# Ezreal11/EaBNet

Hardware: AMD Instinct MI355X
Metric: enhanced frames/sec (16 kHz, 8-mic) at 1/2/4/8 MI355X; RTF per utterance (higher is better)
Workload: dtype f32; 1 GPU; BASELINE configs[1]/[2]: batch of 16 four-second 8-mic 16 kHz utterances per GPU, wave -> STFT+compress -> EaBNet.forward, inference, full hand-written HIP path; batch_per_gpu=16, global_batch=16, mics=8, frames_per_utt=401, freq_bins=161, parallelism=dp1 (independent shards, no collective), pipeline_depth=3

## Files before the change

eabnet_amd/_lib.py:

```python
from __future__ import annotations

import ctypes as C
import os
from typing import Optional

_HERE = os.path.dirname(os.path.abspath(__file__))
LIB_PATH = os.path.join(_HERE, "lib", "libeabnet_hip.so")
ABI_VERSION = 10
MAX_TAPS = 16
_fp = C.POINTER(C.c_float)


class TimeWindow(C.Structure):
    _fields_ = [("pos", C.c_void_p), ("count", C.c_int32), ("lens", C.c_void_p)]


class ConvDesc(C.Structure):
    _fields_ = [
        ("src0", C.c_void_p), ("src1", C.c_void_p), ("xf0", C.c_void_p), ("xf1", C.c_void_p),
        ("slope0", C.c_void_p), ("slope1", C.c_void_p),
        ("C0", C.c_int32), ("C1", C.c_int32), ("xf_mode", C.c_int32),
        ("w", C.c_void_p), ("bias", C.c_void_p),
        ("N", C.c_int32), ("Kpad", C.c_int32),
        ("B", C.c_int32), ("T", C.c_int32), ("Fin", C.c_int32), ("Fout", C.c_int32),
# ... 63 lines not shown
                            + [C.c_void_p] * 4),
    "eab_si_sdr_loss_bwd_f32": (C.c_int, [C.c_void_p, C.c_longlong, C.c_int] * 2 + [C.c_void_p, C.c_int, C.c_void_p, C.c_void_p,
                                          C.c_int, C.c_double, C.c_void_p, C.c_longlong, C.c_void_p]),
    "eab_mrstft_workspace_bytes": (C.c_longlong, [C.c_void_p] + [C.c_int] * 4),
    "eab_mrstft_loss_f32": (C.c_int, [C.c_void_p, C.c_longlong, C.c_int] * 2 + [C.c_void_p, C.c_int, C.c_void_p, C.c_int, C.c_void_p]
                            + [C.c_double] * 3 + [C.c_void_p, C.c_longlong] + [C.c_void_p] * 4),
    "eab_mrstft_loss_bwd_f32": (C.c_int, [C.c_void_p, C.c_longlong, C.c_int] * 2 + [C.c_void_p, C.c_int, C.c_void_p, C.c_int, C.c_void_p,
                                          C.c_double, C.c_void_p, C.c_void_p, C.c_int, C.c_double, C.c_void_p, C.c_longlong,
                                          C.c_void_p, C.c_longlong, C.c_void_p]),
    "eab_norm_act_win_f32": (C.c_int, [C.c_void_p] * 7 + [C.c_int] * 4 + [TimeWindow, C.c_void_p]),
    "eab_lstm64_stream_f32": (C.c_int, [C.c_void_p] * 3 + [C.c_float] + [C.c_void_p] * 4 + [C.c_int] * 4
                              + [TimeWindow, C.c_void_p]),
    "eab_bfw_filter_sum_win_f32": (C.c_int, [C.c_void_p] * 6 + [C.c_int] * 4 + [TimeWindow, C.c_void_p]),
    "eab_mlp_bfw_filter_sum_f32": (C.c_int, [C.c_void_p] * 8 + [C.c_int] * 4 + [TimeWindow, C.c_void_p]),
    "eab_zero_rows_f32": (C.c_int, [C.c_void_p] + [C.c_int] * 3 + [TimeWindow, C.c_void_p]),
    "eab_shift_rows_f32": (C.c_int, [C.c_void_p] + [C.c_int] * 5 + [C.c_void_p]),
    "eab_com_mag_mse_loss_f32": (C.c_int, [C.c_void_p] * 3 + [C.c_int] * 3 + [C.c_void_p, C.c_int, C.c_void_p, C.c_void_p,
                                            C.c_void_p]),
    "eab_energy_ratios_f32": (C.c_int, [C.c_void_p, C.c_longlong, C.c_int] * 3 + [C.c_void_p, C.c_int, C.c_void_p, C.c_int,
                                        C.c_void_p, C.c_void_p]),
    "eab_com_mag_mse_loss_lens_f32": (C.c_int, [C.c_void_p] * 3 + [C.c_int] * 4 + [C.c_void_p, C.c_int, C.c_void_p, C.c_void_p]),
    "eab_stoi_frame_capacity": (C.c_int, [C.c_int]),
    "eab_stoi_workspace_bytes": (C.c_longlong, [C.c_int, C.c_int]),
    "eab_stoi_f32": (C.c_int, [C.c_void_p, C.c_longlong, C.c_int] * 2 + [C.c_void_p, C.c_int, C.c_void_p, C.c_longlong]
                     + [C.c_void_p] * 5),
    "eab_stoi_bwd_workspace_bytes": (C.c_longlong, [C.c_int, C.c_int]),
    "eab_stoi_bwd_f32": (C.c_int, [C.c_void_p, C.c_longlong, C.c_int, C.c_int, C.c_void_p, C.c_int, C.c_void_p, C.c_longlong,
                                   C.c_double, C.c_double, C.c_void_p, C.c_int, C.c_double, C.c_void_p, C.c_longlong, C.c_void_p,
                                   C.c_longlong, C.c_void_p]),
    "eab_resample_bwd_f32": (C.c_int, [C.c_void_p, C.c_longlong, C.c_int, C.c_void_p, C.c_int, C.c_int, C.c_void_p, C.c_longlong,
                                       C.c_int, C.c_void_p, C.c_void_p, C.c_int, C.c_int, C.c_int, C.c_void_p]),
    "eab_resample_f32": (C.c_int, [C.c_void_p, C.c_longlong, C.c_int, C.c_void_p, C.c_void_p, C.c_int, C.c_int,
                                   C.c_void_p, C.c_longlong, C.c_int, C.c_void_p, C.c_void_p, C.c_int, C.c_int, C.c_int,
                                   C.c_longlong, C.c_longlong, C.c_longlong, C.c_void_p]),
    "eab_room_gains_f32": (C.c_int, [C.c_void_p] + [C.c_int] * 3 + [C.c_void_p] * 2 + [C.c_double, C.c_void_p, C.c_int, C.c_void_p,
                                                                                       C.c_void_p]),
    "eab_room_rirs_f32": (C.c_int, [C.c_void_p] + [C.c_int] * 4 + [C.c_double, C.c_void_p, C.c_void_p]),
    "eab_room_rirs_tail_f32": (C.c_int, [C.c_void_p] + [C.c_int] * 4 + [C.c_double, C.c_void_p, C.c_void_p]),
    "eab_room_workspace_bytes": (C.c_longlong, [C.c_int] * 5),
    "eab_room_convolve_f32": (C.c_int, [C.c_void_p] + [C.c_int] * 3 + [C.c_void_p] * 5 + [C.c_int] * 2 + [C.c_void_p] * 2
                              + [C.c_longlong] + [C.c_void_p] * 3),
    "eab_grad_sumsq_f64": (C.c_int, [C.POINTER(OptimSegment), C.c_int, C.c_void_p, C.c_longlong, C.c_void_p]),
    "eab_adam_clip_f32": (C.c_int, [C.POINTER(OptimSegment), C.c_int, C.c_void_p, C.c_longlong] + [C.c_double] * 7
                          + [C.c_void_p, C.c_void_p]),
    "eab_gag_pack_f32": (C.c_int, [C.c_void_p] * 4 + [C.c_int] * 4 + [TimeWindow, C.c_void_p]),
    "eab_gag_crm_f32": (C.c_int, [C.c_void_p] * 6 + [C.c_int] * 6 + [TimeWindow, C.c_void_p]),
    "eab_gag_crm_bwd_f32": (C.c_int, [C.c_void_p] * 9 + [C.c_int] * 6 + [C.c_void_p]),
    "eab_conv_tiles": (C.c_int, [C.c_int] * 3),
    "eab_conv_f32": (C.c_int, [C.POINTER(ConvDesc), C.c_void_p]),
    "eab_train_cln_bwd_f32": (C.c_int, [C.c_void_p] * 11 + [C.c_int] * 5 + [C.c_void_p]),
    "eab_conv_st_chain_plan": (C.c_int, [C.POINTER(ConvDesc), C.c_int, C.POINTER(C.c_int), C.POINTER(C.c_int), C.POINTER(C.c_int)]),
    "eab_conv_st_chain_run": (C.c_int, [C.c_void_p, C.c_void_p, C.c_int, C.c_int, C.c_int, C.c_int, C.c_void_p]),
    "eab_conv_bf16": (C.c_int, [C.POINTER(ConvDesc), C.c_void_p]),
    "eab_lstm64_bf16": (C.c_int, [C.c_void_p] * 3 + [C.c_float] + [C.c_void_p] * 3 + [C.c_int] * 3 + [C.c_void_p]),
    "eab_in_finalize_f32": (C.c_int, [C.c_void_p] + [C.c_int] * 5 + [C.c_float] + [C.c_void_p] * 6 + [C.c_void_p]),
    "eab_norm_act_f32": (C.c_int, [C.c_void_p] * 7 + [C.c_int] * 3 + [C.c_void_p]),
    "eab_lstm64_f32": (C.c_int, [C.c_void_p] * 3 + [C.c_float] + [C.c_void_p] * 3 + [C.c_int] * 3 + [C.c_void_p]),
    "eab_lstm64_prec_f32": (C.c_int, [C.c_void_p] * 3 + [C.c_float] + [C.c_void_p] * 3 + [C.c_int] * 4 + [C.c_void_p]),
    "eab_bfw_filter_sum_f32": (C.c_int, [C.c_void_p] * 6 + [C.c_int] * 4 + [C.c_void_p]),
    "eab_run_program": (C.c_int, [C.POINTER(Op), C.c_int, C.c_void_p]),
    "eab_sizeof_conv_desc": (C.c_int, []),
    "eab_sizeof_op": (C.c_int, []),
    "eab_sizeof_wgrad_desc": (C.c_int, []),
    "eab_gather_f32": (C.c_int, [C.c_void_p] * 4 + [C.c_longlong, C.c_void_p]),
    "eab_train_in_stats_f32": (C.c_int, [C.c_void_p] * 2 + [C.c_int] * 3 + [C.c_float] + [C.c_void_p] * 4 + [C.c_void_p]),
    "eab_train_in1d_f32": (C.c_int, [C.c_void_p] * 2 + [C.c_int] * 3 + [C.c_float] + [C.c_void_p] * 5 + [C.c_void_p]),
    "eab_train_in1d_multi_f32": (C.c_int, [C.c_void_p] * 2 + [C.c_int] * 4 + [C.c_float] + [C.c_void_p] * 5 + [C.c_void_p]),
    "eab_train_norm_bwd_multi_f32": (C.c_int, [C.c_void_p] * 12 + [C.c_int] * 3 + [C.c_void_p]),
    "eab_in_finalize_mr_f32": (C.c_int, [C.c_void_p] + [C.c_int] * 5 + [C.c_float] + [C.c_void_p] * 8 + [C.c_void_p]),
    "eab_train_norm_act_f32": (C.c_int, [C.c_void_p] * 5 + [C.c_int] * 4 + [C.c_void_p]),
    "eab_train_norm_bwd_f32": (C.c_int, [C.c_void_p] * 12 + [C.c_int] * 4 + [C.c_void_p]),
    "eab_glu_bwd_f32": (C.c_int, [C.c_void_p] * 3 + [C.c_longlong, C.c_int, C.c_void_p]),
    "eab_glu_bwd_ex_f32": (C.c_int, [C.c_void_p] * 3 + [C.c_longlong, C.c_int, C.c_int, C.c_void_p]),
    "eab_gate_fwd_f32": (C.c_int, [C.c_void_p] * 3 + [C.c_longlong, C.c_void_p]),
    "eab_gate_bwd_f32": (C.c_int, [C.c_void_p] * 5 + [C.c_longlong, C.c_void_p]),
    "eab_add_f32": (C.c_int, [C.c_void_p] * 3 + [C.c_longlong, C.c_void_p]),
    "eab_copy_f32": (C.c_int, [C.c_void_p] * 2 + [C.c_longlong, C.c_void_p]),
    "eab_relu_bwd_f32": (C.c_int, [C.c_void_p] * 3 + [C.c_longlong, C.c_void_p]),
    "eab_colsum_f32": (C.c_int, [C.c_void_p] * 2 + [C.c_longlong, C.c_int, C.c_void_p]),
    "eab_filter_sum_bwd_f32": (C.c_int, [C.c_void_p] * 3 + [C.c_int] * 5 + [C.c_void_p]),
    "eab_filter_sum_ld_f32": (C.c_int, [C.c_void_p] * 3 + [C.c_int] * 5 + [C.c_void_p]),
    "eab_layernorm64_fwd_f32": (C.c_int, [C.c_void_p] * 3 + [C.c_float] + [C.c_void_p] * 2 + [C.c_longlong, C.c_void_p]),
    "eab_layernorm64_bwd_f32": (C.c_int, [C.c_void_p] * 7 + [C.c_longlong, C.c_void_p]),
    "eab_lstm64_train_fwd_f32": (C.c_int, [C.c_void_p] * 5 + [C.c_int] * 3 + [C.c_void_p]),
    "eab_lstm64_bwd_f32": (C.c_int, [C.c_void_p] * 4 + [C.c_int] * 3 + [C.c_void_p]),
    "eab_lstm64_train_fwd_prec_f32": (C.c_int, [C.c_void_p] * 5 + [C.c_int] * 4 + [C.c_void_p]),
    "eab_lstm64_bwd_prec_f32": (C.c_int, [C.c_void_p] * 4 + [C.c_int] * 4 + [C.c_void_p]),
    "eab_wgrad_f32": (C.c_int, [C.POINTER(WgradDesc), C.c_void_p]),
    "eab_wgrad_batchable": (C.c_int, [C.c_void_p, C.c_int, C.c_int]),
    "eab_wgrad_batch_f32": (C.c_int, [C.c_void_p, C.c_int, C.c_int, C.c_void_p]),
    "eab_lstm64_bwd_form": (C.c_int, [C.c_int] * 4),
    "eab_train_in_stats_lens_f32": (C.c_int, [C.c_void_p] * 2 + [C.c_int] * 3 + [C.c_float] + [C.c_void_p] * 4
                                    + [C.c_void_p, C.c_int, C.c_void_p]),
    "eab_train_in1d_lens_f32": (C.c_int, [C.c_void_p] * 2 + [C.c_int] * 3 + [C.c_float] + [C.c_void_p] * 5
                                + [C.c_void_p, C.c_int, C.c_void_p]),
    "eab_train_in1d_multi_lens_f32": (C.c_int, [C.c_void_p] * 2 + [C.c_int] * 4 + [C.c_float] + [C.c_void_p] * 5
                                      + [C.c_void_p, C.c_int, C.c_void_p]),
    "eab_train_norm_bwd_lens_f32": (C.c_int, [C.c_void_p] * 12 + [C.c_int] * 4 + [C.c_void_p, C.c_int, C.c_void_p]),
    "eab_train_norm_bwd_multi_lens_f32": (C.c_int, [C.c_void_p] * 12 + [C.c_int] * 3 + [C.c_void_p, C.c_int, C.c_void_p]),
    "eab_layernorm64_bwd_lens_f32": (C.c_int, [C.c_void_p] * 7 + [C.c_longlong, C.c_void_p, C.c_int, C.c_int, C.c_void_p]),
    "eab_lstm64_bwd_lens_f32": (C.c_int, [C.c_void_p] * 5 + [C.c_int] * 4 + [C.c_void_p]),
    "eab_filter_sum_ld_lens_f32": (C.c_int, [C.c_void_p] * 3 + [C.c_int] * 5 + [C.c_void_p, C.c_void_p]),
    "eab_wgrad_batch_lens_f32": (C.c_int, [C.c_void_p, C.c_int, C.c_int, C.c_void_p, C.c_void_p]),
    "eab_cln_stats_f32": (C.c_int, [C.c_void_p] * 2 + [C.c_int] * 4 + [C.c_float] + [C.c_void_p] * 3 + [TimeWindow, C.c_void_p]),
    "eab_cln_apply_f32": (C.c_int, [C.c_void_p] * 7 + [C.c_int] * 5 + [TimeWindow, C.c_void_p]),
    "eab_cln_step_f32": (C.c_int, [C.c_void_p] * 10 + [C.c_int] * 5 + [C.c_float, TimeWindow, C.c_void_p]),
# ... 36 lines not shown
```

eabnet_amd/csrc/conv_gemm.hip:

```cpp
#include "device.h"
#include <type_traits>

#define CG_THREADS 256

#define CG_PLAIN 0
#define CG_GLU 1
#define CG_DUAL 2
#define CG_PH2 3
#define CG_XFC 128

#define CG_PMAX 352

template <int MI, int NI, int KU, int MODE, bool PATCH, bool XFT>
struct CgSmem {
    static constexpr int BM = 64 * MI, BN = 64 * NI, LDK = 16 * KU + 4;
    static constexpr int NA = MODE == CG_DUAL ? 2 : 1;
    static constexpr int ATILE = BM * LDK;
    float a[PATCH ? CG_PMAX * LDK : NA * 2 * ATILE];
    float b[2][BN * LDK];
    float xft[2][CG_XFC][2];
    float xsl[2][CG_XFC];
    int dt[EAB_MAX_TAPS];
    int ioff[EAB_MAX_TAPS];
    int last;
    static constexpr int RW = MODE == CG_PH2 ? 2 : 1;
    __attribute__((aligned(16))) unsigned rtab_own[XFT ? BM * RW : 4];
    static_assert(XFT || sizeof(float) * 2 * CG_XFC * 2 >= sizeof(unsigned) * BM * RW, "row table inside xft");
};

__device__ __forceinline__ void cg_merge(float& n, float& mean, float& m2, float nb, float meanb, float m2b) {
    const float nt = n + nb;
    if (nt > 0.0f) {
        const float delta = meanb - mean;
        const float fb = nb / nt;
        mean = fmaf(delta, fb, mean);
        m2 = m2 + m2b + delta * delta * n * fb;
    }
    n = nt;
}

template <int MI, int NI, int KU, int MODE, int XF, bool VEC, int PREC, bool PATCH, bool WIDE = false>
__global__ __launch_bounds__(CG_THREADS, (MI == 2 && NI == 2 && KU == 1 && MODE == CG_GLU) ? 3 : (MODE == CG_PH2 ? 2 : 1)) void conv_gemm_kernel(const eab_conv_desc d) {
    static_assert(MODE != CG_PH2 || (PATCH && NI == 2), "phase-pair form: patch pipeline, one column block per phase and wave");
    static_assert(!PATCH || (KU == 1 && MODE != CG_DUAL && VEC), "patch mode: one unit per stage, single transform");
    constexpr bool H3 = PREC == EAB_PREC_F16X3;
    constexpr bool BF = PREC == EAB_PREC_BF16;
    constexpr bool PH2 = MODE == CG_PH2;
    constexpr bool GLU = MODE != CG_PLAIN;
    constexpr bool DUAL = MODE == CG_DUAL;
    using Smem = CgSmem<MI, NI, KU, MODE, PATCH, XF != EAB_XF_NONE>;
    constexpr int BM = Smem::BM, BN = Smem::BN, LDK = Smem::LDK;
    __shared__ __attribute__((aligned(16))) Smem sm;

    const int tid = threadIdx.x;
    const int lane = tid & 63, wave = tid >> 6;
    const int wm = wave >> 1, wn = wave & 1;
    const int li = lane & 31, lh = lane >> 5;

    const int t_lo = d.win.pos ? *d.win.pos : 0;
    int t_hi = d.win.pos ? (t_lo + d.win.count < d.T ? t_lo + d.win.count : d.T) : d.T;
    const int tiles_per_b = ((d.win.pos ? d.win.count : d.T) * d.No + BM - 1) / BM;
    unsigned vblk = blockIdx.x;
    if (gridDim.x >= 64) {
        const unsigned G = gridDim.x, G8 = G >> 3, rem = G & 7, xcd = vblk & 7, idx = vblk >> 3;
        vblk = xcd * G8 + (xcd < rem ? xcd : rem) + idx;
    }
    const int b = (int)(vblk / (unsigned)tiles_per_b);
    const int tile = (int)vblk - b * tiles_per_b;
    int t_src = d.T;
    if (d.win.lens) {
        t_src = min(t_src, d.win.lens[b]);
        t_hi = min(t_hi, t_src);
    }
    const int Q = t_hi * d.No;
    const int q0 = t_lo * d.No + tile * BM;
    const int n_blk = blockIdx.y * BN;
    const float inv_no = 1.0f / (float)d.No;

#pragma unroll
    for (int j = 0; j < EAB_MAX_TAPS; ++j)
        if (tid == j) {
            sm.dt[j] = d.dt[j];
            sm.ioff[j] = d.ioff[j];
        }

    const int Cout = d.Cout;
    const unsigned row_bytes = (unsigned)(d.Fout * Cout) * 4u, step_bytes = (unsigned)(d.ostride * Cout) * 4u;
    const unsigned phase_bytes = (unsigned)(d.ophase * Cout) * 4u, chan_bytes = (unsigned)Cout * 4u;
    unsigned* const rtab = XF != EAB_XF_NONE ? sm.rtab_own : reinterpret_cast<unsigned*>(&sm.xft[0][0][0]);
    if (tid < BM) {
        const int q = q0 + tid;
        const bool ok = q < Q;
        const int t = eab_div(ok ? q : 0, d.No, inv_no), o = (ok ? q : 0) - t * d.No;
        const unsigned off = ok ? (unsigned)t * row_bytes + (unsigned)o * step_bytes + phase_bytes : EAB_OOB;
        if constexpr (PH2)
            *reinterpret_cast<uint2*>(&rtab[2 * tid]) = make_uint2(off, (ok && 2 * o + 1 < d.Fout) ? off + chan_bytes : EAB_OOB);
        else
            rtab[tid] = off;
    }

    if (XF != EAB_XF_NONE) {
        const int k = tid >> 7, c = tid & (CG_XFC - 1);
        const int Ck = (k == 0 || DUAL) ? d.C0 : d.C1;
        const float* xfk = k == 0 ? d.xf0 : d.xf1;
        const float* slk = k == 0 ? d.slope0 : d.slope1;
        float sc = 1.0f, sh = 0.0f, sl = 1.0f;
        if (c < Ck) {
            if (d.fin_stats && k < d.fin_nsets) {
                const float* gm = k == 0 ? d.fin_gamma0 : d.fin_gamma1;
                const float* bt = k == 0 ? d.fin_beta0 : d.fin_beta1;
                double sn = 0.0, sm = 0.0, sq = 0.0;
                for (int t = 0; t < d.fin_tiles; ++t) {
                    const f32x4 v = *reinterpret_cast<const f32x4*>(
                        &d.fin_stats[((((size_t)b * d.fin_tiles + t) * d.fin_nsets + k) * d.C0 + c) * 4]);
                    const double n = (double)v[0], mu = (double)v[1];
                    sn += n;
                    sm = fma(n, mu, sm);
                    sq += fma(n * mu, mu, (double)v[2]);
                }
                const double mean = sn > 0.0 ? sm / sn : 0.0;
                double var = sn > 0.0 ? sq / sn - mean * mean : 0.0;
                if (var < 0.0) var = 0.0;
                const double scale = (double)gm[c] / sqrt(var + (double)d.fin_eps);
                sc = (float)scale;
                sh = (float)((double)bt[c] - mean * scale);
                sl = slk[c];
            } else if (xfk) {
                const float2 v = *reinterpret_cast<const float2*>(&xfk[((size_t)b * Ck + c) * 2]);
                sc = v.x;
                sh = v.y;
                sl = slk[c];
            }
        }
        sm.xft[k][c][0] = sc;
        sm.xft[k][c][1] = sh;
        sm.xsl[k][c] = sl;
    }

    const int Ctot = d.C0 + d.C1;
    const int UPT = (Ctot + 15) >> 4;
    const int NU = d.ntaps * UPT;
    static_assert(!WIDE || (PREC == EAB_PREC_BF16 && KU == 1 && VEC && !PATCH && XF == EAB_XF_NONE && MODE != CG_DUAL), "WIDE: see above");
    constexpr bool w0 = WIDE, w1 = WIDE;
    const int NS = (w0 || w1) ? d.ntaps * ((w0 ? d.C0 >> 5 : (d.C0 + 15) >> 4) + (d.C1 > 0 ? (w1 ? d.C1 >> 5 : (d.C1 + 15) >> 4) : 0))
                              : (NU + KU - 1) / KU;

    constexpr unsigned esz0 = WIDE ? 2u : 4u, esz1 = WIDE ? 2u : 4u;
    const unsigned bytes0 = (unsigned)d.T * d.Fin * d.C0 * esz0;
    const unsigned bytes1 = (unsigned)d.T * d.Fin * d.C1 * esz1;
    const __amdgpu_buffer_rsrc_t rs0 = __builtin_amdgcn_make_buffer_rsrc(
        const_cast<char*>(reinterpret_cast<const char*>(d.src0)) + (size_t)b * bytes0, 0, bytes0, 0x00020000);
    const __amdgpu_buffer_rsrc_t rs1 = __builtin_amdgcn_make_buffer_rsrc(
        const_cast<char*>(reinterpret_cast<const char*>(d.src1 ? d.src1 : d.src0)) + (d.src1 ? (size_t)b * bytes1 : 0), 0,
        d.src1 ? bytes1 : 0u, 0x00020000);

    const int srow = tid >> 2;
    const int skq = tid & 3;
    const float* wrow[NI];
#pragma unroll
    for (int p = 0; p < NI; ++p) wrow[p] = d.w + (size_t)(n_blk + srow + 64 * p) * d.Kpad + skq * 4;

    f32x16 acc[MI][NI];
#pragma unroll
    for (int mi = 0; mi < MI; ++mi)
#pragma unroll
        for (int ni = 0; ni < NI; ++ni)
#pragma unroll
            for (int r = 0; r < 16; ++r) acc[mi][ni][r] = 0.0f;

    auto lds_barrier = [] { asm volatile("s_waitcnt lgkmcnt(0)\n\ts_barrier" ::: "memory"); };

    __syncthreads();

    if (q0 < Q) {
    if constexpr (PATCH) {
        constexpr int PP = (CG_PMAX + 63) / 64;
        int dt_min = 0, io_min = 0, io_max = 0;
#pragma unroll
        for (int j = 0; j < EAB_MAX_TAPS; ++j)
            if (j < d.ntaps) {
                dt_min = d.dt[j] < dt_min ? d.dt[j] : dt_min;
                io_min = d.ioff[j] < io_min ? d.ioff[j] : io_min;
                io_max = d.ioff[j] > io_max ? d.ioff[j] : io_max;
            }
        const int halo_lo = -io_min;
        const int hi_need = (d.No - 1) * d.istride + io_max - (d.Fin - 1);
        const int Fp = d.Fin + halo_lo + (hi_need > 0 ? hi_need : 0);
        const float inv_fp = 1.0f / (float)Fp;
        const int t_first = eab_div(q0, d.No, inv_no);
        const int t_last = eab_div((q0 + BM < Q ? q0 + BM : (Q > q0 ? Q : q0 + 1)) - 1, d.No, inv_no);
        const int P = (t_last - t_first + 1 - dt_min) * Fp;

        const int d64 = eab_div(64, Fp, inv_fp), m64 = 64 - d64 * Fp;
        int p_tf[PP];
        bool p_ok[PP], p_all[PP];
        {
            const int tr = eab_div(srow, Fp, inv_fp);
            int f = srow - tr * Fp, t_in = t_first + dt_min + tr;
            int tf = t_in * d.Fin + f - halo_lo;
#pragma unroll
            for (int pp = 0; pp < PP; ++pp) {
                p_ok[pp] = p_all[pp] = false;
                p_tf[pp] = 0;
                if (64 * pp < P) {
                    p_ok[pp] = srow + 64 * pp < P && (unsigned)t_in < (unsigned)t_src && (unsigned)(f - halo_lo) < (unsigned)d.Fin;
                    if (XF != EAB_XF_NONE) p_all[pp] = __builtin_amdgcn_ballot_w64(p_ok[pp]) == __builtin_amdgcn_ballot_w64(true);
                    p_tf[pp] = tf;
                    f += m64;
                    t_in += d64;
                    tf += d64 * d.Fin + m64;
                    if (f >= Fp) {
                        f -= Fp;
                        ++t_in;
                        tf += d.Fin - Fp;
                    }
                }
            }
        }
        int fa[MI];
#pragma unroll
        for (int mi = 0; mi < MI; ++mi) {
            int q = q0 + (wm * MI + mi) * 32 + li;
            q = q < Q ? q : (Q > q0 ? Q - 1 : q0);
            const int t = eab_div(q, d.No, inv_no), o = q - t * d.No;
            fa[mi] = ((t - t_first - dt_min) * Fp + o * d.istride + halo_lo) * LDK + 4 * lh;
        }
        const int b_base = (wn * NI * 32 + li) * LDK + 4 * lh;

        f32x4 rp[PP];
        f32x4 rbw0[NI], rbw1[NI];
        int p_tc = 0;
        auto patch_fetch = [&](int chunk) {
            const int c0 = chunk << 4;
            const bool second = (d.C1 > 0) && (c0 >= d.C0);
            const int Cs = second ? d.C1 : d.C0;
            const int c = (second ? c0 - d.C0 : c0) + skq * 4;
            const bool cok = c < Cs;
            p_tc = ((second ? 1 : 0) << 8) | (cok ? c : 0);
#pragma unroll
            for (int pp = 0; pp < PP; ++pp) {
                if (64 * pp >= P) continue;
                const unsigned off = (p_ok[pp] && cok) ? (unsigned)((p_tf[pp] * Cs + c) * 4) : EAB_OOB;
                const u32x4 v = second ? __builtin_amdgcn_raw_buffer_load_b128(rs1, off, 0, 0)
                                       : __builtin_amdgcn_raw_buffer_load_b128(rs0, off, 0, 0);
                rp[pp] = __builtin_bit_cast(f32x4, v);
            }
// ... 764 lines not shown
                    cg_merge(n, mu, q, red[i1], red[i1 + 1], red[i1 + 2]);
                    *reinterpret_cast<f32x4*>(&d.stats[((tbase + s) * Cout + ch[c]) * 4]) = f32x4{n, mu, q, 0.0f};
                }
            }
        }
        if (d.fz_counter) {
            __threadfence();
            __syncthreads();
            if (tid == 0) sm.last = atomicAdd(&d.fz_counter[b], 1) == d.stat_tiles - 1;
            __syncthreads();
            if (sm.last) {
                __threadfence();
                const int nch = d.nsets * Cout;
                const int NSL = CG_THREADS / nch;
                const int e = tid % nch, slice = tid / nch;
                const int s = e / Cout, c = e - s * Cout;
                double* dred = reinterpret_cast<double*>(&sm.a[0]);
                double sn = 0.0, sm_ = 0.0, sq = 0.0;
                if (slice < NSL) {
                    const float* p = d.stats + (((size_t)b * d.stat_tiles) * d.nsets + s) * Cout * 4 + (size_t)c * 4;
                    const size_t stride = (size_t)d.nsets * Cout * 4;
                    for (int t = slice; t < d.stat_tiles; t += NSL) {
                        const f32x4 v = *reinterpret_cast<const f32x4*>(p + (size_t)t * stride);
                        const double n = (double)v[0], mu = (double)v[1];
                        sn += n;
                        sm_ = fma(n, mu, sm_);
                        sq += fma(n * mu, mu, (double)v[2]);
                    }
                    dred[(0 * NSL + slice) * nch + e] = sn;
                    dred[(1 * NSL + slice) * nch + e] = sm_;
                    dred[(2 * NSL + slice) * nch + e] = sq;
                }
                __syncthreads();
                if (slice == 0) {
                    sn = sm_ = sq = 0.0;
                    for (int k = 0; k < NSL; ++k) {
                        sn += dred[(0 * NSL + k) * nch + e];
                        sm_ += dred[(1 * NSL + k) * nch + e];
                        sq += dred[(2 * NSL + k) * nch + e];
                    }
                    const double mean = sn > 0.0 ? sm_ / sn : 0.0;
                    double var = sn > 0.0 ? sq / sn - mean * mean : 0.0;
                    if (var < 0.0) var = 0.0;
                    const float* gm = s == 0 ? d.fz_gamma0 : d.fz_gamma1;
                    const float* bt = s == 0 ? d.fz_beta0 : d.fz_beta1;
                    float* xf = s == 0 ? d.fz_xf0 : d.fz_xf1;
                    const double scale = (double)gm[c] / sqrt(var + (double)d.fz_eps);
                    *reinterpret_cast<float2*>(&xf[((size_t)b * Cout + c) * 2]) = make_float2((float)scale, (float)((double)bt[c] - mean * scale));
                }
                if (tid == 0) d.fz_counter[b] = 0;
            }
        }
    }
}

extern "C" int eab_conv_tiles(int T, int No, int bm) {
    if (T <= 0 || No <= 0 || (bm != 16 && bm != 32 && bm != 64 && bm != 128)) return -1;
    long long q = (long long)T * No;
    return (int)((q + bm - 1) / bm);
}

int eab_conv_st(const eab_conv_desc* d, hipStream_t s);

template <int MI, int NI, int KU, int MODE, int XF, bool VEC>
static int cg_launch(const eab_conv_desc* d, hipStream_t s) {
    constexpr int BM = 64 * MI, BN = 64 * NI;
    const int tiles = eab_conv_tiles(d->win.pos ? d->win.count : d->T, d->No, BM);
    dim3 grid((unsigned)(d->B * tiles), (unsigned)(d->N / BN));
    constexpr bool can_patch = KU == 1 && MODE != CG_DUAL && VEC && XF != EAB_XF_PRELU_NORM;
    if (d->korder == EAB_KORDER_CHUNK) {
        if constexpr (can_patch) {
            if (d->precision == EAB_PREC_F16X3)
                hipLaunchKernelGGL((conv_gemm_kernel<MI, NI, 1, MODE, XF, true, EAB_PREC_F16X3, true>), grid,
                                   dim3(CG_THREADS), 0, s, *d);
            else if (d->precision == EAB_PREC_BF16)
                hipLaunchKernelGGL((conv_gemm_kernel<MI, NI, 1, MODE, XF, true, EAB_PREC_BF16, true>), grid,
                                   dim3(CG_THREADS), 0, s, *d);
            else
                hipLaunchKernelGGL((conv_gemm_kernel<MI, NI, 1, MODE, XF, true, EAB_PREC_F32, true>), grid,
                                   dim3(CG_THREADS), 0, s, *d);
            EAB_RETURN_LAUNCH_STATUS();
        } else {
            return EAB_EUNSUPPORTED;
        }
    }
    if constexpr (MODE == CG_PH2) {
        return EAB_EUNSUPPORTED;
    } else {
    if (d->precision == EAB_PREC_F16X3) {
        if constexpr (VEC)
            hipLaunchKernelGGL((conv_gemm_kernel<MI, NI, KU, MODE, XF, VEC, EAB_PREC_F16X3, false>), grid,
                               dim3(CG_THREADS), 0, s, *d);
        else
            return EAB_EUNSUPPORTED;
    } else if (d->precision == EAB_PREC_BF16) {
        if constexpr (VEC) {
            if (d->src_bf16) {
                if constexpr (KU == 1 && XF == EAB_XF_NONE && MODE != CG_DUAL)
                    hipLaunchKernelGGL((conv_gemm_kernel<MI, NI, KU, MODE, XF, VEC, EAB_PREC_BF16, false, true>), grid,
                                       dim3(CG_THREADS), 0, s, *d);
                else
                    return EAB_EUNSUPPORTED;
            } else {
                hipLaunchKernelGGL((conv_gemm_kernel<MI, NI, KU, MODE, XF, VEC, EAB_PREC_BF16, false>), grid,
                                   dim3(CG_THREADS), 0, s, *d);
            }
        } else {
            return EAB_EUNSUPPORTED;
        }
    } else {
        hipLaunchKernelGGL((conv_gemm_kernel<MI, NI, KU, MODE, XF, VEC, EAB_PREC_F32, false>), grid, dim3(CG_THREADS), 0,
                           s, *d);
    }
    EAB_RETURN_LAUNCH_STATUS();
    }
}

static long long cg_patch_positions(const eab_conv_desc* d) {
    int dt_min = 0, io_min = 0, io_max = 0;
    for (int j = 0; j < d->ntaps; ++j) {
        dt_min = d->dt[j] < dt_min ? d->dt[j] : dt_min;
        io_min = d->ioff[j] < io_min ? d->ioff[j] : io_min;
        io_max = d->ioff[j] > io_max ? d->ioff[j] : io_max;
    }
    const int hi_need = (d->No - 1) * d->istride + io_max - (d->Fin - 1);
    const long long Fp = d->Fin - io_min + (hi_need > 0 ? hi_need : 0);
    const long long rows = (d->bm - 1) / d->No + 2 - dt_min;
    return rows * Fp;
}

template <int MI, int NI, int MODE, int XF, bool VEC>
static int cg_pick_ku(const eab_conv_desc* d, hipStream_t s, int ku) {
    if (ku == 4) {
        if constexpr (MI == 1 && MODE != CG_GLU && VEC) return cg_launch<MI, NI, 4, MODE, XF, VEC>(d, s);
        return EAB_EUNSUPPORTED;
    }
    if (ku == 2) {
        if constexpr (VEC && MODE != CG_DUAL) return cg_launch<MI, NI, 2, MODE, XF, VEC>(d, s);
        return EAB_EUNSUPPORTED;
    }
    return cg_launch<MI, NI, 1, MODE, XF, VEC>(d, s);
}

extern "C" int eab_conv_f32(const eab_conv_desc* d, eab_stream_t stream) {
    EAB_CHECK_ARG(d && d->src0 && d->w && d->dst);
    EAB_CHECK_ARG(d->B > 0 && d->T > 0 && d->Fin > 0 && d->Fout > 0 && d->No > 0);
    EAB_CHECK_ARG(d->C0 > 0 && d->C1 >= 0 && (d->C1 == 0) == (d->src1 == nullptr));
    EAB_CHECK_ARG(d->C1 == 0 || (d->C0 % 16) == 0);
    EAB_CHECK_ARG(d->ntaps > 0 && d->ntaps <= EAB_MAX_TAPS);
    EAB_CHECK_ARG(d->ostride >= 1 && d->istride >= 1 && d->ophase >= 0 && d->ophase < d->ostride);
    EAB_CHECK_ARG((d->No - 1) * d->ostride + d->ophase < d->Fout);
    const int upt = (d->C0 + d->C1 + 15) / 16;
    EAB_CHECK_ARG(d->Kpad == d->ntaps * upt * 16);
    for (int j = 0; j < d->ntaps; ++j) {
        EAB_CHECK_ARG(d->dt[j] < (1 << 20) && d->dt[j] > -(1 << 20));
        EAB_CHECK_ARG(d->dt[j] <= 0 || d->korder != EAB_KORDER_CHUNK);
    }
    EAB_CHECK_ARG(d->epi >= EAB_EPI_LINEAR && d->epi <= EAB_EPI_PHASE2);
    EAB_CHECK_ARG(d->precision == EAB_PREC_F32 || d->precision == EAB_PREC_F16X3 || d->precision == EAB_PREC_BF16);
    EAB_CHECK_ARG(d->korder == EAB_KORDER_TAP || d->korder == EAB_KORDER_CHUNK || d->korder == EAB_KORDER_FRAG);
    EAB_CHECK_ARG(d->korder == EAB_KORDER_FRAG || d->ph1_No == 0);
    if (d->korder == EAB_KORDER_CHUNK) {
        EAB_CHECK_ARG(cg_patch_positions(d) <= CG_PMAX && d->epi != EAB_EPI_DUALGATE);
        EAB_CHECK_ARG(d->C0 % 4 == 0 && d->C1 % 4 == 0 && d->xf_mode != EAB_XF_PRELU_NORM);
    }
    if (d->win.pos) {
        EAB_CHECK_ARG(d->win.count > 0 && d->stats == nullptr && d->fin_stats == nullptr);
// ... 46 lines not shown
    }
    if (d->stats) {
        const int tiles = eab_conv_tiles(d->T, d->No, d->bm) + (d->ph1_No > 0 ? eab_conv_tiles(d->T, d->ph1_No, d->bm) : 0);
        EAB_CHECK_ARG(d->stat_tile0 >= 0 && d->stat_tile0 + tiles <= d->stat_tiles);
    }
    EAB_CHECK_ARG((long long)d->B * (eab_conv_tiles(d->T, d->No, d->bm) + (d->ph1_No > 0 ? eab_conv_tiles(d->T, d->ph1_No, d->bm) : 0)) < (1ll << 31));
    hipStream_t s = eab_stream(stream);
    if (d->korder == EAB_KORDER_FRAG) return eab_conv_st(d, s);
    const int mi = d->bm / 64;
    const bool vec = (d->C0 % 4 == 0) && (d->C1 % 4 == 0);
    const bool has_xf = d->xf_mode != EAB_XF_NONE && (d->xf0 || d->xf1 || fin);
    const int xf = has_xf ? d->xf_mode : EAB_XF_NONE;
    if (xf != EAB_XF_NONE)
        EAB_CHECK_ARG(d->C0 <= CG_XFC && d->C1 <= CG_XFC && vec);
    int ku = (mi == 1 && !glu && vec && d->Fin == 1) ? 4 : 1;
    if (d->korder == EAB_KORDER_CHUNK) ku = 1;
    if (ku == 4 && !(mi == 1 && !glu && vec)) ku = 1;
    if (ku == 2 && (!vec || dual)) ku = 1;
    if (ph2) {
        if (!vec || xf == EAB_XF_PRELU_NORM) return EAB_EUNSUPPORTED;
        if (xf == EAB_XF_NORM_PRELU)
            return mi == 2 ? cg_launch<2, 2, 1, CG_PH2, EAB_XF_NORM_PRELU, true>(d, s) : cg_launch<1, 2, 1, CG_PH2, EAB_XF_NORM_PRELU, true>(d, s);
        return mi == 2 ? cg_launch<2, 2, 1, CG_PH2, EAB_XF_NONE, true>(d, s) : cg_launch<1, 2, 1, CG_PH2, EAB_XF_NONE, true>(d, s);
    }
    if (dual) {
        if (d->N != 128 || mi != 1 || xf != EAB_XF_PRELU_NORM) return EAB_EUNSUPPORTED;
        return cg_pick_ku<1, 2, CG_DUAL, EAB_XF_PRELU_NORM, true>(d, s, ku == 2 ? 1 : ku);
    }
    if (glu) {
        if (d->N % 128 != 0 || xf == EAB_XF_PRELU_NORM) return EAB_EUNSUPPORTED;
        if (!vec) return mi == 2 ? cg_pick_ku<2, 2, CG_GLU, 0, false>(d, s, 1) : cg_pick_ku<1, 2, CG_GLU, 0, false>(d, s, 1);
        if (xf == EAB_XF_NORM_PRELU)
            return mi == 2 ? cg_pick_ku<2, 2, CG_GLU, EAB_XF_NORM_PRELU, true>(d, s, ku)
                           : cg_pick_ku<1, 2, CG_GLU, EAB_XF_NORM_PRELU, true>(d, s, ku);
        return mi == 2 ? cg_pick_ku<2, 2, CG_GLU, 0, true>(d, s, ku) : cg_pick_ku<1, 2, CG_GLU, 0, true>(d, s, ku);
    }
    if (!vec) return EAB_EUNSUPPORTED;
#define CG_DISPATCH_XF(MI_, NI_)                                                           \
    (xf == EAB_XF_NONE        ? cg_pick_ku<MI_, NI_, CG_PLAIN, EAB_XF_NONE, true>(d, s, ku) \
     : xf == EAB_XF_NORM_PRELU ? cg_pick_ku<MI_, NI_, CG_PLAIN, EAB_XF_NORM_PRELU, true>(d, s, ku) \
                               : cg_pick_ku<MI_, NI_, CG_PLAIN, EAB_XF_PRELU_NORM, true>(d, s, ku))
    if (d->N % 128 == 0) return mi == 2 ? CG_DISPATCH_XF(2, 2) : CG_DISPATCH_XF(1, 2);
    if (d->N % 64 == 0) return mi == 2 ? CG_DISPATCH_XF(2, 1) : CG_DISPATCH_XF(1, 1);
#undef CG_DISPATCH_XF
    return EAB_EUNSUPPORTED;
}

extern "C" int eab_conv_bf16(const eab_conv_desc* d, eab_stream_t stream) {
    EAB_CHECK_ARG(d);
    eab_conv_desc dd = *d;
    dd.precision = EAB_PREC_BF16;
    return eab_conv_f32(&dd, stream);
}
```

include/eabnet_hip.h:

```cpp
#ifndef EABNET_HIP_H
#define EABNET_HIP_H

#include <stdint.h>

#ifdef __cplusplus
extern "C" {
#endif

#define EAB_ABI_VERSION 10

#define EAB_OK          0
#define EAB_EINVAL      1
#define EAB_EUNSUPPORTED 2
#define EAB_EHIP_BASE   1000

typedef void* eab_stream_t;

int         eab_abi_version(void);
const char* eab_error_string(int code);

typedef struct eab_time_window {
    const int32_t* pos;
    int32_t count;
    const int32_t* lens;
// ... 141 lines not shown
    float* dst;
    float* dst_acc;
    int32_t Cout;
    float* stats;
    int32_t nsets;
    const float* stat_slope0;
    const float* stat_slope1;
    int32_t stat_tiles;
    int32_t stat_tile0;
    int32_t bm;
    const float* fin_stats;
    const float* fin_gamma0;
    const float* fin_beta0;
    const float* fin_gamma1;
    const float* fin_beta1;
    int32_t fin_tiles, fin_nsets, fin_count;
    float fin_eps;
    int32_t precision;
    int32_t korder;
    eab_time_window win;
    int32_t* fz_counter;
    const float* fz_gamma0;
    const float* fz_beta0;
    float* fz_xf0;
    const float* fz_gamma1;
    const float* fz_beta1;
    float* fz_xf1;
    float fz_eps;
    float* glu_dump;
    const float* ph1_w;
    int32_t ph1_No, ph1_ophase, ph1_ntaps, ph1_Kpad;
    int32_t ph1_dt[EAB_MAX_TAPS];
    int32_t ph1_ioff[EAB_MAX_TAPS];
    const float* f2_w;
    float* f2_dst;
    float* f2_stats;
    const float* f2_stat_slope0;
    const float* f2_stat_slope1;
    int32_t f2_N, f2_nsets, f2_stat_tiles;
    int32_t p2_mask1;
    int32_t src_bf16;
} eab_conv_desc;

#define EAB_PREC_F32   0
#define EAB_PREC_F16X3 1
#define EAB_PREC_BF16  2
#define EAB_KORDER_TAP   0
#define EAB_KORDER_CHUNK 1
#define EAB_KORDER_FRAG  2

int eab_conv_tiles(int T, int No, int bm);
int eab_conv_f32(const eab_conv_desc* d, eab_stream_t stream);
int eab_conv_bf16(const eab_conv_desc* d, eab_stream_t stream);

int eab_in_finalize_f32(const float* stats, int B, int C, int nsets, int stat_tiles,
                        int count , float eps,
                        const float* gamma0, const float* beta0, float* xf0,
                        const float* gamma1, const float* beta1, float* xf1,
                        eab_stream_t stream);

int eab_norm_act_f32(const float* a, const float* xfa, const float* slopea,
                     const float* b, const float* xfb, const float* slopeb,
                     float* out, int B, int P, int C, eab_stream_t stream);

int eab_lstm64_f32(const float* x, const float* ln_g, const float* ln_b, float ln_eps,
                   const float* wcat, const float* bias, float* h_out,
                   int B, int T, int F, eab_stream_t stream);
int eab_lstm64_prec_f32(const float* x, const float* ln_g, const float* ln_b, float ln_eps,
                        const float* wcat, const float* bias, float* h_out,
                        int B, int T, int F, int precision, eab_stream_t stream);
int eab_lstm64_bf16(const float* x, const float* ln_g, const float* ln_b, float ln_eps,
                    const float* wcat, const float* bias, float* h_out, int B, int T, int F, eab_stream_t stream);

int eab_bfw_filter_sum_f32(const float* y1, const float* w2, const float* b2, const float* x,
                           float* out, float* bfw, int B, int T, int F, int M,
                           eab_stream_t stream);

#define EAB_OP_CONV        1
#define EAB_OP_IN_FINALIZE 2
#define EAB_OP_NORM_ACT    3
#define EAB_OP_LSTM64      4
#define EAB_OP_BFW_FS      5
#define EAB_OP_MEMSET0     6
#define EAB_OP_GAG_PACK    7
#define EAB_OP_GAG_CRM     8
#define EAB_OP_CONV_CHAIN  9

typedef struct eab_wgrad_desc {
    const float* dz;
    const float* src0;
    const float* src1;
    float* dw;
    float* dbias;
    int32_t N, C0, C1, Kpad;
    int32_t B, T, Fin, Fz, No, ostride, ophase, istride;
    int32_t ntaps;
    int32_t dt[EAB_MAX_TAPS];
    int32_t ioff[EAB_MAX_TAPS];
    int32_t rows_per_wg;
    int32_t precision;
    int32_t bf16_mask;
} eab_wgrad_desc;

typedef struct eab_op {
    int32_t kind;
    int32_t i[8];
// ... 157 lines not shown
```

Baseline: 994,400 frames/s.

## Make phase-pair conv GEMM kernel persistent with grid-stride tile loop

For the phase-pair (CG_PH2, KU=1) conv kernel, the launch grid is capped at the number of resident workgroup slots (occupancy × CU count). Each workgroup then loops over tiles in an XCD-aware strided order, hoisting the tap tables, patch geometry and per-batch transform loads out of the loop. The aim is to cut workgroup launch and prologue overhead and to reuse the transform setup across tiles. In exchange it adds a loop with extra barriers and asm opacity tricks that may raise register pressure, and it may rebalance the tail poorly. Runtime knobs and a grid-size probe API are also added.

```diff
diff --git a/eabnet_amd/_lib.py b/eabnet_amd/_lib.py
--- a/eabnet_amd/_lib.py
+++ b/eabnet_amd/_lib.py
@@ -139,6 +139,8 @@
     "eab_conv_st_chain_plan": (C.c_int, [C.POINTER(ConvDesc), C.c_int, C.POINTER(C.c_int), C.POINTER(C.c_int), C.POINTER(C.c_int)]),
     "eab_conv_st_chain_run": (C.c_int, [C.c_void_p, C.c_void_p, C.c_int, C.c_int, C.c_int, C.c_int, C.c_void_p]),
     "eab_conv_bf16": (C.c_int, [C.POINTER(ConvDesc), C.c_void_p]),
+    "eab_conv_resident": (C.c_int, [C.c_int, C.c_int]),
+    "eab_conv_grid_x": (C.c_int, [C.POINTER(ConvDesc)]),
     "eab_lstm64_bf16": (C.c_int, [C.c_void_p] * 3 + [C.c_float] + [C.c_void_p] * 3 + [C.c_int] * 3 + [C.c_void_p]),
     "eab_in_finalize_f32": (C.c_int, [C.c_void_p] + [C.c_int] * 5 + [C.c_float] + [C.c_void_p] * 6 + [C.c_void_p]),
     "eab_norm_act_f32": (C.c_int, [C.c_void_p] * 7 + [C.c_int] * 3 + [C.c_void_p]),
diff --git a/eabnet_amd/csrc/conv_gemm.hip b/eabnet_amd/csrc/conv_gemm.hip
--- a/eabnet_amd/csrc/conv_gemm.hip
+++ b/eabnet_amd/csrc/conv_gemm.hip
@@ -1,4 +1,5 @@
 #include "device.h"
+#include <atomic>
 #include <type_traits>
 
 #define CG_THREADS 256
@@ -39,8 +40,29 @@
     n = nt;
 }
 
+template <int KU, int MODE>
+constexpr bool cg_resident() { return KU == 1 && MODE == CG_PH2; }
+
+template <bool RES>
+__device__ __forceinline__ decltype(auto) cg_desc(const eab_conv_desc& d) {
+    if constexpr (RES) {
+        auto p = (const __attribute__((address_space(4))) eab_conv_desc*)__builtin_amdgcn_kernarg_segment_ptr();
+        asm volatile("" : "+s"(p));
+        return *p;
+    } else {
+        return d;
+    }
+}
+
+template <bool RES, typename T>
+__device__ __forceinline__ T cg_opaque(T v) {
+    if constexpr (RES) asm volatile("" : "+v"(v));
+    return v;
+}
+
 template <int MI, int NI, int KU, int MODE, int XF, bool VEC, int PREC, bool PATCH, bool WIDE = false>
-__global__ __launch_bounds__(CG_THREADS, (MI == 2 && NI == 2 && KU == 1 && MODE == CG_GLU) ? 3 : (MODE == CG_PH2 ? 2 : 1)) void conv_gemm_kernel(const eab_conv_desc d) {
+__global__ __launch_bounds__(CG_THREADS, (MI == 2 && NI == 2 && KU == 1 && MODE == CG_GLU) ? 3 : (MODE == CG_PH2 ? 2 : 1)) void conv_gemm_kernel(const eab_conv_desc d_arg) {
+    const eab_conv_desc& d = d_arg;
     static_assert(MODE != CG_PH2 || (PATCH && NI == 2), "phase-pair form: patch pipeline, one column block per phase and wave");
     static_assert(!PATCH || (KU == 1 && MODE != CG_DUAL && VEC), "patch mode: one unit per stage, single transform");
     constexpr bool H3 = PREC == EAB_PREC_F16X3;
@@ -48,23 +70,76 @@
     constexpr bool PH2 = MODE == CG_PH2;
     constexpr bool GLU = MODE != CG_PLAIN;
     constexpr bool DUAL = MODE == CG_DUAL;
+    constexpr bool RES = cg_resident<KU, MODE>();
     using Smem = CgSmem<MI, NI, KU, MODE, PATCH, XF != EAB_XF_NONE>;
     constexpr int BM = Smem::BM, BN = Smem::BN, LDK = Smem::LDK;
     __shared__ __attribute__((aligned(16))) Smem sm;
 
-    const int tid = threadIdx.x;
-    const int lane = tid & 63, wave = tid >> 6;
-    const int wm = wave >> 1, wn = wave & 1;
-    const int li = lane & 31, lh = lane >> 5;
+    const int tid0 = threadIdx.x;
+    const int lane0 = tid0 & 63, wave0 = tid0 >> 6;
+    const int wm0 = wave0 >> 1, wn0 = wave0 & 1;
+    const int li0 = lane0 & 31, lh0 = lane0 >> 5;
 
     const int t_lo = d.win.pos ? *d.win.pos : 0;
-    int t_hi = d.win.pos ? (t_lo + d.win.count < d.T ? t_lo + d.win.count : d.T) : d.T;
+    const int t_hi_win = d.win.pos ? (t_lo + d.win.count < d.T ? t_lo + d.win.count : d.T) : d.T;
     const int tiles_per_b = ((d.win.pos ? d.win.count : d.T) * d.No + BM - 1) / BM;
-    unsigned vblk = blockIdx.x;
-    if (gridDim.x >= 64) {
+    unsigned vblk = blockIdx.x, v_end = blockIdx.x + 1, v_step = 1;
+    if constexpr (RES) {
+        const unsigned G = (unsigned)(d.B * tiles_per_b), W = gridDim.x;
+        v_end = G;
+        v_step = W;
+        if (G >= 64 && W >= 8) {
+            const unsigned G8 = G >> 3, rem = G & 7, xcd = vblk & 7, idx = vblk >> 3;
+            const unsigned first = xcd * G8 + (xcd < rem ? xcd : rem);
+            vblk = first + idx;
+            v_end = first + G8 + (xcd < rem ? 1u : 0u);
+            v_step = (W >> 3) + (xcd < (W & 7) ? 1u : 0u);
+        }
+    } else if (gridDim.x >= 64) {
         const unsigned G = gridDim.x, G8 = G >> 3, rem = G & 7, xcd = vblk & 7, idx = vblk >> 3;
         vblk = xcd * G8 + (xcd < rem ? xcd : rem) + idx;
     }
+
+    if constexpr (RES) {
+#pragma unroll
+        for (int j = 0; j < EAB_MAX_TAPS; ++j)
+            if (tid0 == j) {
+                sm.dt[j] = d.dt[j];
+                sm.ioff[j] = d.ioff[j];
+            }
+    }
+
+    auto lds_barrier = [] { asm volatile("s_waitcnt lgkmcnt(0)\n\ts_barrier" ::: "memory"); };
+
+    constexpr int PP = (CG_PMAX + 63) / 64;
+    int w_dt_min = 0, w_halo_lo = 0, w_Fp = 1, w_d64 = 0, w_m64 = 0;
+    float w_inv_fp = 1.0f;
+    if constexpr (RES) {
+        int io_min = 0, io_max = 0;
+#pragma unroll
+        for (int j = 0; j < EAB_MAX_TAPS; ++j)
+            if (j < d.ntaps) {
+                w_dt_min = d.dt[j] < w_dt_min ? d.dt[j] : w_dt_min;
+                io_min = d.ioff[j] < io_min ? d.ioff[j] : io_min;
+                io_max = d.ioff[j] > io_max ? d.ioff[j] : io_max;
+            }
+        w_halo_lo = -io_min;
+        const int hi_need = (d.No - 1) * d.istride + io_max - (d.Fin - 1);
+        w_Fp = d.Fin + w_halo_lo + (hi_need > 0 ? hi_need : 0);
+        w_inv_fp = 1.0f / (float)w_Fp;
+        w_d64 = eab_div(64, w_Fp, w_inv_fp);
+        w_m64 = 64 - w_d64 * w_Fp;
+    }
+
+    int b_tab = -1;
+    if (RES && vblk >= v_end) return;
+    for (;;) {
+    const auto& d = cg_desc<RES>(d_arg);
+    const int tid = cg_opaque<RES>(tid0);
+    const int lane = RES ? tid & 63 : lane0, wave = RES ? tid >> 6 : wave0;
+    const int wm = RES ? wave >> 1 : wm0, wn = RES ? wave & 1 : wn0;
+    const int li = RES ? lane & 31 : li0, lh = RES ? lane >> 5 : lh0;
+    int t_hi = t_hi_win;
     const int b = (int)(vblk / (unsigned)tiles_per_b);
     const int tile = (int)vblk - b * tiles_per_b;
     int t_src = d.T;
@@ -77,12 +152,14 @@
     const int n_blk = blockIdx.y * BN;
     const float inv_no = 1.0f / (float)d.No;
 
-#pragma unroll
-    for (int j = 0; j < EAB_MAX_TAPS; ++j)
-        if (tid == j) {
-            sm.dt[j] = d.dt[j];
-            sm.ioff[j] = d.ioff[j];
-        }
+    if constexpr (!RES) {
+#pragma unroll
+        for (int j = 0; j < EAB_MAX_TAPS; ++j)
+            if (tid == j) {
+                sm.dt[j] = d.dt[j];
+                sm.ioff[j] = d.ioff[j];
+            }
+    }
 
     const int Cout = d.Cout;
     const unsigned row_bytes = (unsigned)(d.Fout * Cout) * 4u, step_bytes = (unsigned)(d.ostride * Cout) * 4u;
@@ -99,7 +176,8 @@
             rtab[tid] = off;
     }
 
-    if (XF != EAB_XF_NONE) {
+    if (XF != EAB_XF_NONE && (!RES || b != b_tab)) {
+        b_tab = b;
         const int k = tid >> 7, c = tid & (CG_XFC - 1);
         const int Ck = (k == 0 || DUAL) ? d.C0 : d.C1;
         const float* xfk = k == 0 ? d.xf0 : d.xf1;
@@ -144,10 +222,10 @@
     constexpr bool w0 = WIDE, w1 = WIDE;
     const int NS = (w0 || w1) ? d.ntaps * ((w0 ? d.C0 >> 5 : (d.C0 + 15) >> 4) + (d.C1 > 0 ? (w1 ? d.C1 >> 5 : (d.C1 + 15) >> 4) : 0))
                               : (NU + KU - 1) / KU;
-
     constexpr unsigned esz0 = WIDE ? 2u : 4u, esz1 = WIDE ? 2u : 4u;
     const unsigned bytes0 = (unsigned)d.T * d.Fin * d.C0 * esz0;
     const unsigned bytes1 = (unsigned)d.T * d.Fin * d.C1 * esz1;
+
     const __amdgpu_buffer_rsrc_t rs0 = __builtin_amdgcn_make_buffer_rsrc(
         const_cast<char*>(reinterpret_cast<const char*>(d.src0)) + (size_t)b * bytes0, 0, bytes0, 0x00020000);
     const __amdgpu_buffer_rsrc_t rs1 = __builtin_amdgcn_make_buffer_rsrc(
@@ -161,21 +239,21 @@
     for (int p = 0; p < NI; ++p) wrow[p] = d.w + (size_t)(n_blk + srow + 64 * p) * d.Kpad + skq * 4;
 
     f32x16 acc[MI][NI];
+    const float zero = cg_opaque<RES>(0.0f);
 #pragma unroll
     for (int mi = 0; mi < MI; ++mi)
 #pragma unroll
         for (int ni = 0; ni < NI; ++ni)
 #pragma unroll
-            for (int r = 0; r < 16; ++r) acc[mi][ni][r] = 0.0f;
-
-    auto lds_barrier = [] { asm volatile("s_waitcnt lgkmcnt(0)\n\ts_barrier" ::: "memory"); };
-
-    __syncthreads();
+            for (int r = 0; r < 16; ++r) acc[mi][ni][r] = zero;
+
+    if constexpr (RES) lds_barrier();
+    else __syncthreads();
 
     if (q0 < Q) {
     if constexpr (PATCH) {
-        constexpr int PP = (CG_PMAX + 63) / 64;
-        int dt_min = 0, io_min = 0, io_max = 0;
+        int dt_min = RES ? w_dt_min : 0, io_min = 0, io_max = 0;
+        if constexpr (!RES) {
 #pragma unroll
         for (int j = 0; j < EAB_MAX_TAPS; ++j)
             if (j < d.ntaps) {
@@ -183,15 +261,16 @@
                 io_min = d.ioff[j] < io_min ? d.ioff[j] : io_min;
                 io_max = d.ioff[j] > io_max ? d.ioff[j] : io_max;
             }
-        const int halo_lo = -io_min;
+        }
+        const int halo_lo = RES ? w_halo_lo : -io_min;
         const int hi_need = (d.No - 1) * d.istride + io_max - (d.Fin - 1);
-        const int Fp = d.Fin + halo_lo + (hi_need > 0 ? hi_need : 0);
-        const float inv_fp = 1.0f / (float)Fp;
+        const int Fp = RES ? w_Fp : d.Fin + halo_lo + (hi_need > 0 ? hi_need : 0);
+        const float inv_fp = RES ? w_inv_fp : 1.0f / (float)Fp;
         const int t_first = eab_div(q0, d.No, inv_no);
         const int t_last = eab_div((q0 + BM < Q ? q0 + BM : (Q > q0 ? Q : q0 + 1)) - 1, d.No, inv_no);
         const int P = (t_last - t_first + 1 - dt_min) * Fp;
 
-        const int d64 = eab_div(64, Fp, inv_fp), m64 = 64 - d64 * Fp;
+        const int d64 = RES ? w_d64 : eab_div(64, Fp, inv_fp), m64 = RES ? w_m64 : 64 - d64 * Fp;
         int p_tf[PP];
         bool p_ok[PP], p_all[PP];
         {
@@ -1062,6 +1141,14 @@
             }
         }
     }
+    if constexpr (!RES) {
+        break;
+    } else {
+        vblk += v_step;
+        if (vblk >= v_end) break;
+        lds_barrier();
+    }
+    }
 }
 
 extern "C" int eab_conv_tiles(int T, int No, int bm) {
@@ -1071,6 +1158,54 @@
 }
 
 int eab_conv_st(const eab_conv_desc* d, hipStream_t s);
+
+static std::atomic<int> cg_res_on{1}, cg_res_max_wgs{0};
+static thread_local int* cg_grid_probe = nullptr;
+
+extern "C" int eab_conv_resident(int on, int max_wgs) {
+    EAB_CHECK_ARG((on == 0 || on == 1) && max_wgs >= 0);
+    cg_res_on.store(on);
+    cg_res_max_wgs.store(max_wgs);
+    return EAB_OK;
+}
+
+template <auto KERNEL>
+static int cg_device_slots(int* slots) {
+    constexpr int NDEV = 16;
+    static std::atomic<int> cached[NDEV];
+    int dev = 0;
+    if (hipError_t e = hipGetDevice(&dev); e != hipSuccess) return eab_hip_status(e);
+    int n = (dev >= 0 && dev < NDEV) ? cached[dev].load(std::memory_order_relaxed) : 0;
+    if (n == 0) {
+        int per_cu = 0, cus = 0;
+        if (hipError_t e = hipOccupancyMaxActiveBlocksPerMultiprocessor(&per_cu, KERNEL, CG_THREADS, 0); e != hipSuccess) return eab_hip_status(e);
+        if (hipError_t e = hipDeviceGetAttribute(&cus, hipDeviceAttributeMultiprocessorCount, dev); e != hipSuccess) return eab_hip_status(e);
+        if (per_cu <= 0 || cus <= 0) return EAB_EUNSUPPORTED;
+        n = per_cu * cus;
+        if (dev >= 0 && dev < NDEV) cached[dev].store(n, std::memory_order_relaxed);
+    }
+    *slots = n;
+    return EAB_OK;
+}
+
+template <auto KERNEL, bool RES>
+static int cg_enqueue(dim3 grid, const eab_conv_desc* d, hipStream_t s) {
+    if constexpr (RES) {
+        if (cg_res_on.load() && !d->win.pos) {
+            int slots = 0;
+            const int cap = cg_res_max_wgs.load();
+            if (cap > 0) slots = cap;
+            else if (int rc = cg_device_slots<KERNEL>(&slots); rc != EAB_OK) return rc;
+            if ((unsigned)slots < grid.x) grid.x = (unsigned)slots;
+        }
+    }
+    if (cg_grid_probe) {
+        *cg_grid_probe = (int)grid.x;
+        return EAB_OK;
+    }
+    hipLaunchKernelGGL(KERNEL, grid, dim3(CG_THREADS), 0, s, *d);
+    EAB_RETURN_LAUNCH_STATUS();
+}
 
 template <int MI, int NI, int KU, int MODE, int XF, bool VEC>
 static int cg_launch(const eab_conv_desc* d, hipStream_t s) {
@@ -1081,15 +1216,11 @@
     if (d->korder == EAB_KORDER_CHUNK) {
         if constexpr (can_patch) {
             if (d->precision == EAB_PREC_F16X3)
-                hipLaunchKernelGGL((conv_gemm_kernel<MI, NI, 1, MODE, XF, true, EAB_PREC_F16X3, true>), grid,
-                                   dim3(CG_THREADS), 0, s, *d);
+                return cg_enqueue<conv_gemm_kernel<MI, NI, 1, MODE, XF, true, EAB_PREC_F16X3, true>, cg_resident<1, MODE>()>(grid, d, s);
             else if (d->precision == EAB_PREC_BF16)
-                hipLaunchKernelGGL((conv_gemm_kernel<MI, NI, 1, MODE, XF, true, EAB_PREC_BF16, true>), grid,
-                                   dim3(CG_THREADS), 0, s, *d);
+                return cg_enqueue<conv_gemm_kernel<MI, NI, 1, MODE, XF, true, EAB_PREC_BF16, true>, cg_resident<1, MODE>()>(grid, d, s);
             else
-                hipLaunchKernelGGL((conv_gemm_kernel<MI, NI, 1, MODE, XF, true, EAB_PREC_F32, true>), grid,
-                                   dim3(CG_THREADS), 0, s, *d);
-            EAB_RETURN_LAUNCH_STATUS();
+                return cg_enqueue<conv_gemm_kernel<MI, NI, 1, MODE, XF, true, EAB_PREC_F32, true>, cg_resident<1, MODE>()>(grid, d, s);
         } else {
             return EAB_EUNSUPPORTED;
         }
@@ -1099,30 +1230,25 @@
     } else {
     if (d->precision == EAB_PREC_F16X3) {
         if constexpr (VEC)
-            hipLaunchKernelGGL((conv_gemm_kernel<MI, NI, KU, MODE, XF, VEC, EAB_PREC_F16X3, false>), grid,
-                               dim3(CG_THREADS), 0, s, *d);
+            return cg_enqueue<conv_gemm_kernel<MI, NI, KU, MODE, XF, VEC, EAB_PREC_F16X3, false>, cg_resident<KU, MODE>()>(grid, d, s);
         else
             return EAB_EUNSUPPORTED;
     } else if (d->precision == EAB_PREC_BF16) {
         if constexpr (VEC) {
             if (d->src_bf16) {
                 if constexpr (KU == 1 && XF == EAB_XF_NONE && MODE != CG_DUAL)
-                    hipLaunchKernelGGL((conv_gemm_kernel<MI, NI, KU, MODE, XF, VEC, EAB_PREC_BF16, false, true>), grid,
-                                       dim3(CG_THREADS), 0, s, *d);
+                    return cg_enqueue<conv_gemm_kernel<MI, NI, KU, MODE, XF, VEC, EAB_PREC_BF16, false, true>, cg_resident<KU, MODE>()>(grid, d, s);
                 else
                     return EAB_EUNSUPPORTED;
             } else {
-                hipLaunchKernelGGL((conv_gemm_kernel<MI, NI, KU, MODE, XF, VEC, EAB_PREC_BF16, false>), grid,
-                                   dim3(CG_THREADS), 0, s, *d);
+                return cg_enqueue<conv_gemm_kernel<MI, NI, KU, MODE, XF, VEC, EAB_PREC_BF16, false>, cg_resident<KU, MODE>()>(grid, d, s);
             }
         } else {
             return EAB_EUNSUPPORTED;
         }
     } else {
-        hipLaunchKernelGGL((conv_gemm_kernel<MI, NI, KU, MODE, XF, VEC, EAB_PREC_F32, false>), grid, dim3(CG_THREADS), 0,
-                           s, *d);
-    }
-    EAB_RETURN_LAUNCH_STATUS();
+        return cg_enqueue<conv_gemm_kernel<MI, NI, KU, MODE, XF, VEC, EAB_PREC_F32, false>, cg_resident<KU, MODE>()>(grid, d, s);
+    }
     }
 }
 
@@ -1275,3 +1401,12 @@
     dd.precision = EAB_PREC_BF16;
     return eab_conv_f32(&dd, stream);
 }
+
+extern "C" int eab_conv_grid_x(const eab_conv_desc* d) {
+    if (!d || d->korder == EAB_KORDER_FRAG) return -1;
+    int gx = -1;
+    cg_grid_probe = &gx;
+    const int rc = eab_conv_f32(d, nullptr);
+    cg_grid_probe = nullptr;
+    return rc == EAB_OK ? gx : -1;
+}
diff --git a/include/eabnet_hip.h b/include/eabnet_hip.h
--- a/include/eabnet_hip.h
+++ b/include/eabnet_hip.h
@@ -217,6 +217,8 @@
 int eab_conv_tiles(int T, int No, int bm);
 int eab_conv_f32(const eab_conv_desc* d, eab_stream_t stream);
 int eab_conv_bf16(const eab_conv_desc* d, eab_stream_t stream);
+int eab_conv_resident(int on, int max_wgs);
+int eab_conv_grid_x(const eab_conv_desc* d);
 
 int eab_in_finalize_f32(const float* stats, int B, int C, int nsets, int stat_tiles,
                         int count , float eps,
```

Measured after the change: 990,000 frames/s. No clear change (-0.4%).
